# ActiveVisionLab/nope-nerf

Hardware: AMD Instinct MI355X
Metric: training rays/sec (higher is better)
Workload: dtype f32; 1 GPU; BASELINE configs[1]: 1024 rays/GPU x 192 samples, D=256, fp32 via three fp16 MFMA terms per product (fwd, dgrad, wgrad 4x4 + encoding tiles); fp32_products=split2, adam_arithmetic=single, rays_per_gpu=1024, total_rays=1024, n_samples=192, hidden=256, parallelism=dp1 (ray-sharded, one flat all-reduce)

## Files before the change

nope-nerf_amd/csrc/nnr_wgrad.hip:

```cpp
#include "nnr_device.h"
#include "nnr_kernels.h"
#include "nnr_split.h"
#include <cstdlib>

namespace nnr {

NNR_TL_DECL(tl_wgrad)
#ifdef NNR_TIMELINE
__device__ unsigned long long tl_wgrad_all[4096];
extern "C" int nnr_timeline_wgrad_all(unsigned long long* host4096) {
    return (int)hipMemcpyFromSymbol(host4096, HIP_SYMBOL(tl_wgrad_all), 4096 * sizeof(unsigned long long));
}
#endif

template <int W>
struct Vec { float v[W]; };

template <int W>
__device__ __forceinline__ Vec<W> load_vec(const float* p) {
    Vec<W> r;
    if constexpr (W == 4) {
        const f32x4 t = *reinterpret_cast<const f32x4*>(p);
        r.v[0] = t[0]; r.v[1] = t[1]; r.v[2] = t[2]; r.v[3] = t[3];
    } else if constexpr (W == 2) {
        const f32x2 t = *reinterpret_cast<const f32x2*>(p);
        r.v[0] = t[0]; r.v[1] = t[1];
    } else {
        r.v[0] = *p;
    }
    return r;
}

constexpr int kU = 4;
constexpr int32_t kPlanMagic = 0x4e4e5235;

template <int MI, int NI, int BIAS>
__device__ __forceinline__ void wgrad_job(const WgradJob& jb, const WgradArgs& a, int lane, int ji) {
    const int half = lane >> 5, m = lane & 31;
    const int dp = a.plane_pitch[jb.d_plane], xp = a.plane_pitch[jb.x_plane];
    const bool dok = MI * m < jb.d_valid, xok = NI * m < jb.x_valid;
    const bool dt = a.plane_tile[jb.d_plane] != 0, xt = a.plane_tile[jb.x_plane] != 0;
    const int dc = jb.d_col0 + (dok ? MI * m : 0), xc = jb.x_col0 + (xok ? NI * m : 0);
    const int d_row = dt ? 4 : dp, x_row = xt ? 4 : xp;
    const int64_t d_chunk = 32 * (int64_t)dp, x_chunk = 32 * (int64_t)xp;
    const float* dptr = a.ws + a.plane_off[jb.d_plane] + (dt ? (dc >> 3) * 256 + ((dc >> 2) & 1) * 128 + (dc & 3) : dc) + half * d_row;
    const float* xptr = a.ws + a.plane_off[jb.x_plane] + (xt ? (xc >> 3) * 256 + ((xc >> 2) & 1) * 128 + (xc & 3) : xc) + half * x_row;

    f32x16 acc[MI][NI];
#pragma unroll
    for (int i = 0; i < MI; ++i)
#pragma unroll
        for (int j = 0; j < NI; ++j)
#pragma unroll
            for (int r = 0; r < 16; ++r) acc[i][j][r] = 0.f;
    float bsum[MI];
#pragma unroll
    for (int i = 0; i < MI; ++i) bsum[i] = 0.f;

    Vec<MI> dA[kU], dB[kU];
    Vec<NI> xA[kU], xB[kU];
    auto load_stage = [&](Vec<MI>(&d)[kU], Vec<NI>(&x)[kU], int64_t kk) {
        const float* const dk = dptr + (kk >> 5) * d_chunk + (kk & 31) * d_row;
        const float* const xk = xptr + (kk >> 5) * x_chunk + (kk & 31) * x_row;
#pragma unroll
        for (int u = 0; u < kU; ++u) {
            d[u] = load_vec<MI>(dk + 2 * u * d_row);
            x[u] = load_vec<NI>(xk + 2 * u * x_row);
        }
    };
    auto compute = [&](const Vec<MI>(&d)[kU], const Vec<NI>(&x)[kU]) {
#pragma unroll
        for (int u = 0; u < kU; ++u) {
#pragma unroll
            for (int i = 0; i < MI; ++i) {
#pragma unroll
                for (int j = 0; j < NI; ++j) acc[i][j] = mfma32(d[u].v[i], x[u].v[j], acc[i][j]);
                if (BIAS == 1 || (BIAS == 2 && u % 2 == 0) || (BIAS == 3 && u % 2 == 1)) bsum[i] += d[u].v[i];
            }
        }
    };
    NNR_STAMP(tl_wgrad, 0);
    load_stage(dA, xA, jb.k0);
    for (int64_t k = jb.k0; k < jb.k1; k += 4 * kU) {
        load_stage(dB, xB, k + 2 * kU);
        __builtin_amdgcn_sched_barrier(0);
        compute(dA, xA);
        __builtin_amdgcn_sched_barrier(0);
        load_stage(dA, xA, (k + 4 * kU < jb.k1) ? k + 4 * kU : k);
        __builtin_amdgcn_sched_barrier(0);
        compute(dB, xB);
        __builtin_amdgcn_sched_barrier(0);
    }

    NNR_STAMP(tl_wgrad, 1);
#ifdef NNR_TIMELINE
    if (blockIdx.x == 700 / 8 && threadIdx.x == 0) { tl_wgrad[4] = (unsigned long long)(jb.k1 - jb.k0); tl_wgrad[5] = MI * 8 + NI; }
#endif
    float* slot = a.slots + (int64_t)ji * kSlotFloats;
#pragma unroll
    for (int i = 0; i < MI; ++i)
#pragma unroll
        for (int r = 0; r < 16; ++r) {
            const int mr = (r & 3) + 8 * (r >> 2) + 4 * half;
            float* dst = slot + (MI * mr + i) * (32 * NI) + NI * m;
            if constexpr (NI == 4) *reinterpret_cast<f32x4*>(dst) = f32x4{acc[i][0][r], acc[i][1][r], acc[i][2][r], acc[i][3][r]};
            else if constexpr (NI == 2) *reinterpret_cast<f32x2*>(dst) = f32x2{acc[i][0][r], acc[i][1][r]};
            else *dst = acc[i][0][r];
        }
    if constexpr (BIAS != 0) {
        float* dst = slot + kSlotTile + half * (32 * MI) + MI * m;
#pragma unroll
        for (int i = 0; i < MI; ++i) dst[i] = bsum[i];
    }
    NNR_STAMP(tl_wgrad, 2);
}

constexpr int kStageF4 = 2 * 16 * 64;

template <int BIAS, int NI, bool DTILE, bool XTILE>
__device__ __forceinline__ void wgrad_job_split(const WgradJob& jb, const WgradArgs& a, int lane, int ji, f32x4* stage) {
    constexpr int MI = 4;
    static_assert(NI == 4 || NI == 2, "activation sub-tiles per job");
    static_assert(!XTILE || NI == 4, "the tile-major activation image is laid out for whole 128-column tiles");
    constexpr int G = 6 * NI;
    static_assert(G >= 16, "block 3 issues the 16 DMA rows of the step after next, one per gap");
    const int half = lane >> 5, m = lane & 31;
    const int dp = a.plane_pitch[jb.d_plane], xp = a.plane_pitch[jb.x_plane];
    const bool dok = MI * m < jb.d_valid, xok = NI * m < jb.x_valid;
    const char* const dg = reinterpret_cast<const char*>(a.ws + a.plane_off[jb.d_plane] + (DTILE ? (jb.d_col0 >> 3) * 256 : jb.d_col0));
    const char* const xg = reinterpret_cast<const char*>(a.ws + a.plane_off[jb.x_plane] + (XTILE ? (jb.x_col0 >> 3) * 256 : jb.x_col0));
    const int tlane = ((lane & 15) >> 1) * 1024 + (lane & 1) * 512 + (lane >> 4) * 16;
    const int dlane = DTILE ? tlane : 4 * ((dok ? MI * m : 0) + 8 * half * dp);
    const int64_t d_chunk_bytes = 128 * (int64_t)dp, x_chunk_bytes = 128 * (int64_t)xp;
    const int xlane = XTILE ? tlane : NI == 4 ? 4 * ((xok ? NI * m : 0) + 8 * half * xp) : 4 * (4 * (m & 15) + 8 * half * xp);

    f32x16 acc[MI][NI];
#pragma unroll
    for (int i = 0; i < MI; ++i)
#pragma unroll
        for (int j = 0; j < NI; ++j)
#pragma unroll
            for (int r = 0; r < 16; ++r) acc[i][j][r] = 0.f;
    float bsum[MI] = {0.f, 0.f, 0.f, 0.f};
    uint32_t Xc[NI][3][4], Xn[NI][3][4], Dq[2][3][4];
    f32x2 fp[2][4];
    const float* const lrow = reinterpret_cast<const float*>(stage) + 4 * lane;
    const float* const lrowd = DTILE ? reinterpret_cast<const float*>(stage) + 4 * (256 * half + 64 * (m >> 4) + (m & 15)) : lrow;
    const float* const lrowx = XTILE ? reinterpret_cast<const float*>(stage) + 4 * (256 * half + 64 * (m >> 4) + (m & 15)) + 2048
                             : NI == 4 ? lrow : reinterpret_cast<const float*>(stage) + 4 * (32 * half + (m >> 1)) + 2 * (m & 1);

#define NNR_WDMA(G, LANE, P, KK, S, DST, ROW) \
    __builtin_amdgcn_global_load_lds((glb_ptr_t)((G) + ((KK) + (S)) * (int64_t)(P) * 4 + (LANE)), (lds_ptr_t)((DST) + (ROW) * 64), 16, 0, 0)
#define NNR_WPACK(V) __builtin_bit_cast(uint32_t, __builtin_convertvector(V, bf16x2))
#define NNR_WOFF(ROW0, P, C, SECOND) (((ROW0) == 0 ? DTILE : XTILE) ? 512 * ((P) >> 1) + 128 * ((P) & 1) + (C) + 64 * (SECOND) : 256 * ((ROW0) + 2 * (P) + (SECOND)) + (C))
#define NNR_WFETCH(W, P, LR, ROW0, C) (fp[W][P] = f32x2{(LR)[NNR_WOFF(ROW0, P, C, 0)], (LR)[NNR_WOFF(ROW0, P, C, 1)]})
#define NNR_WDMA_D(KK, S, DST, ROW)                                                                                                      \
    do {                                                                                                                                 \
        if constexpr (DTILE)                                                                                                             \
            __builtin_amdgcn_global_load_lds((glb_ptr_t)(dg + ((KK) >> 5) * d_chunk_bytes + ((KK) & 31) * 16 + ((S) & 1) * 8192 + ((S) >> 1) * 64 + dlane), \
                                             (lds_ptr_t)((DST) + (ROW) * 64), 16, 0, 0);                                                 \
        else NNR_WDMA(dg, dlane, dp, KK, S, DST, ROW);                                                                                    \
    } while (0)
#define NNR_WDMA_X(KK, S, DST, ROW)                                                                                                      \
    do {                                                                                                                                 \
        if constexpr (XTILE)                                                                                                             \
            __builtin_amdgcn_global_load_lds((glb_ptr_t)(xg + ((KK) >> 5) * x_chunk_bytes + ((KK) & 31) * 16 + ((S) & 1) * 8192 + ((S) >> 1) * 64 + xlane), \
                                             (lds_ptr_t)((DST) + (ROW) * 64), 16, 0, 0);                                                 \
        else NNR_WDMA(xg, xlane, xp, KK, S, DST, ROW);                                                                                    \
    } while (0)
#define NNR_WSPLIT(LR, ROW0, C, P, ST, Q, W, BI, BWT)                                        \
    do {                                                                                     \
        if ((ST) == 0) {                                                                     \
            NNR_WFETCH(W, P, LR, ROW0, C);                                                   \
        } else if ((ST) == 1) {                                                              \
            if ((BI) >= 0 && BIAS != 0)                                                      \
                bsum[(BI) >= 0 ? (BI) : 0] += (BWT) * (BIAS == 1 ? fp[W][P][0] + fp[W][P][1] : (BIAS == 2 ? fp[W][P][0] : fp[W][P][1])); \
            Q[2][P] = NNR_WPACK(fp[W][P]);                                   \
            fp[W][P] = pair_residual(fp[W][P], Q[2][P]);                                      \
        } else if ((ST) == 2) {                                                              \
            Q[1][P] = NNR_WPACK(fp[W][P]);                                   \
            fp[W][P] = pair_residual(fp[W][P], Q[1][P]);                                      \
        } else {                                                                             \
            Q[0][P] = NNR_WPACK(fp[W][P]);                                   \
        }                                                                                    \
    } while (0)
#define NNR_WSPLIT_ALL(LR, ROW0, C, Q, W, BI)                                                \
    _Pragma("unroll") for (int st_ = 0; st_ < 4; ++st_)                                      \
        _Pragma("unroll") for (int p_ = 0; p_ < 4; ++p_) NNR_WSPLIT(LR, ROW0, C, p_, st_, Q, W, BI, 1.f)

#pragma unroll
    for (int s = 0; s < 8; ++s) {
        NNR_WDMA_D((int64_t)jb.k0, s, stage, s);
        NNR_WDMA_X((int64_t)jb.k0, s, stage, 8 + s);
    }
    asm volatile("s_waitcnt vmcnt(0)" ::: "memory");
    {
        const int64_t k1st = jb.k0 + 16 < jb.k1 ? jb.k0 + 16 : jb.k0;
#pragma unroll
        for (int s = 0; s < 8; ++s) {
            NNR_WDMA_D(k1st, s, stage + 1024, s);
            NNR_WDMA_X(k1st, s, stage + 1024, 8 + s);
        }
    }
#pragma unroll
    for (int j = 0; j < NI; ++j) NNR_WSPLIT_ALL(lrowx, 8, j, Xc[j], 1, -1);
    NNR_WSPLIT_ALL(lrowd, 0, 0, Dq[0], 0, 0);

    for (int64_t k = jb.k0; k < jb.k1; k += 16) {
        const int par = (int)(((k - jb.k0) >> 4) & 1);
        const bool more = k + 16 < jb.k1;
        const int64_t kn = k + 32 < jb.k1 ? k + 32 : k;
        const float nf = more ? 1.f : 0.f;
        const float* const lc = lrowd + 4096 * par;
        const float* const ln = lrowd + 4096 * (1 - par);
        const float* const lnx = lrowx + 4096 * (1 - par);
        f32x4* const dst = stage + 1024 * par;
#pragma unroll
        for (int i = 0; i < MI; ++i) {
            if (i == 2) asm volatile("s_waitcnt vmcnt(0)" ::: "memory");
            constexpr int kXOps = 16 * (NI / 2);
            const int n_ops = 16 + (i >= 2 ? kXOps : 0);
            const int stride = n_ops / 16;
#pragma unroll
            for (int g = 0; g < G; ++g) {
                const int j = g / 6, t = g % 6;
                const int wc = t == 0 ? 0 : (t < 3 ? 1 : 2), xc = t == 0 ? 2 : (t == 1 ? 1 : (t == 2 ? 2 : t - 3));
                __builtin_amdgcn_sched_barrier(0);
                acc[i][j] = __builtin_amdgcn_mfma_f32_32x32x16_bf16(
                    __builtin_bit_cast(bf16x8, u32x4{Dq[i & 1][wc][0], Dq[i & 1][wc][1], Dq[i & 1][wc][2], Dq[i & 1][wc][3]}),
                    __builtin_bit_cast(bf16x8, u32x4{Xc[j][xc][0], Xc[j][xc][1], Xc[j][xc][2], Xc[j][xc][3]}),
                    acc[i][j], 0, 0, 0);
                __builtin_amdgcn_sched_barrier(0);
                {
                    const int q = i == 3 ? g : 16;
                    if (q < 8) NNR_WDMA_D(kn, q, dst, q);
                    else if (q < 16) NNR_WDMA_X(kn, q - 8, dst, q);
                }
#pragma unroll
                for (int o = 0; o < 48; ++o) {
                    if (o >= n_ops || (o * G) / n_ops != g) continue;
                    const bool is_d = stride == 1 || o % stride == 0;
                    const int od = stride == 1 ? o : o / stride, ox = o - o / stride - 1;
                    if (is_d) {
                        const int st = od / 4, p = od % 4;
                        if (i == 0) NNR_WSPLIT(lc, 0, 1, p, st, Dq[1], 0, 1, 1.f);
                        else if (i == 1) NNR_WSPLIT(lc, 0, 2, p, st, Dq[0], 0, 2, 1.f);
                        else if (i == 2) NNR_WSPLIT(lc, 0, 3, p, st, Dq[1], 0, 3, 1.f);
                        else NNR_WSPLIT(ln, 0, 0, p, st, Dq[0], 0, 0, nf);
                    } else {
                        const int cc = (NI / 2) * (i - 2) + ox / 16, r = ox % 16, st = r / 4, p = r % 4;
                        NNR_WSPLIT(lnx, 8, cc, p, st, Xn[cc], 1, -1, 0.f);
                    }
                }
            }
            if constexpr (NI == 4) asm volatile("" : "+a"(acc[i][0]), "+a"(acc[i][1]), "+a"(acc[i][2]), "+a"(acc[i][3]));
            else asm volatile("" : "+a"(acc[i][0]), "+a"(acc[i][1]));
        }
#pragma unroll
        for (int j = 0; j < NI; ++j)
#pragma unroll
            for (int t = 0; t < 3; ++t)
#pragma unroll
                for (int q = 0; q < 4; ++q) Xc[j][t][q] = Xn[j][t][q];
    }
    asm volatile("s_waitcnt vmcnt(0)" ::: "memory");
#undef NNR_WDMA
#undef NNR_WDMA_D
#undef NNR_WDMA_X
#undef NNR_WOFF
#undef NNR_WSPLIT
#undef NNR_WFETCH
#undef NNR_WPACK
#undef NNR_WSPLIT_ALL

    float* slot = a.slots + (int64_t)ji * kSlotFloats;
#pragma unroll
    for (int i = 0; i < MI; ++i)
#pragma unroll
        for (int r = 0; r < 16; ++r) {
            const int mr = (r & 3) + 8 * (r >> 2) + 4 * half;
            float* dst = slot + (MI * mr + i) * (32 * NI) + NI * m;
            if constexpr (NI == 4) *reinterpret_cast<f32x4*>(dst) = f32x4{acc[i][0][r], acc[i][1][r], acc[i][2][r], acc[i][3][r]};
            else *reinterpret_cast<f32x2*>(dst) = f32x2{acc[i][0][r], acc[i][1][r]};
        }
    if (jb.bias != 0) {
        float* dst = slot + kSlotTile + half * (32 * MI) + MI * m;
#pragma unroll
        for (int i = 0; i < MI; ++i) dst[i] = bsum[i];
    }
}

constexpr int kCoopStageF4 = 2 * 8 * 64;
constexpr int kCoopRegionF4 = 4 * 3 * 64;
constexpr int kCoopXchF4 = kWavesPerBlock * kCoopStageF4;
constexpr int kCoopF4 = kCoopXchF4 + 2 * 4 * kCoopRegionF4;

template <bool DTILE, bool XTILE>
__device__ __forceinline__ void wgrad_group_split(const WgradJob& jb, const WgradArgs& a, int lane, int ji, f32x4* lds_all, int wave) {
    constexpr int MI = 4, NI = 4;
    typedef uint32_t u32x2 __attribute__((ext_vector_type(2)));
    const int half = lane >> 5, m = lane & 31;
    const int ta = __builtin_amdgcn_readfirstlane(jb.d_col0 >> 7), tb = __builtin_amdgcn_readfirstlane(jb.x_col0 >> 7);
    const int dp = a.plane_pitch[jb.d_plane], xp = a.plane_pitch[jb.x_plane];
    f32x4* const stage = lds_all + wave * kCoopStageF4;
    const char* const dg = reinterpret_cast<const char*>(a.ws + a.plane_off[jb.d_plane] + (DTILE ? (jb.d_col0 >> 3) * 256 : jb.d_col0));
    const char* const xg = reinterpret_cast<const char*>(a.ws + a.plane_off[jb.x_plane] + (XTILE ? (jb.x_col0 >> 3) * 256 : jb.x_col0));
    const int tlane = ((lane & 15) >> 1) * 1024 + (lane & 1) * 512 + (lane >> 4) * 16;
    const int dlane = DTILE ? tlane : 4 * (MI * m + 8 * half * dp);
    const int xlane = XTILE ? tlane : 4 * (NI * m + 8 * half * xp);
    const int64_t d_chunk_bytes = 128 * (int64_t)dp, x_chunk_bytes = 128 * (int64_t)xp;
    auto dma_d = [&](int64_t KK, int r, f32x4* dst) __attribute__((always_inline)) {
        if constexpr (DTILE)
            __builtin_amdgcn_global_load_lds((glb_ptr_t)(dg + (KK >> 5) * d_chunk_bytes + (KK & 31) * 16 + (r & 1) * 8192 + (tb + 2 * (r >> 1)) * 64 + dlane),
                                             (lds_ptr_t)(dst + r * 64), 16, 0, 0);
        else
            __builtin_amdgcn_global_load_lds((glb_ptr_t)(dg + (KK + 4 * tb + r) * (int64_t)dp * 4 + dlane), (lds_ptr_t)(dst + r * 64), 16, 0, 0);
    };
    auto dma_x = [&](int64_t KK, int r, f32x4* dst) __attribute__((always_inline)) {
        if constexpr (XTILE)
            __builtin_amdgcn_global_load_lds((glb_ptr_t)(xg + (KK >> 5) * x_chunk_bytes + (KK & 31) * 16 + (r & 1) * 8192 + (ta + 2 * (r >> 1)) * 64 + xlane),
                                             (lds_ptr_t)(dst + (4 + r) * 64), 16, 0, 0);
        else
            __builtin_amdgcn_global_load_lds((glb_ptr_t)(xg + (KK + 4 * ta + r) * (int64_t)xp * 4 + xlane), (lds_ptr_t)(dst + (4 + r) * 64), 16, 0, 0);
    };
    const float* const sf = reinterpret_cast<const float*>(stage);
    const float* const lrd = DTILE ? sf + 4 * (128 * half + 64 * (m >> 4) + (m & 15)) : sf + 4 * lane;
    const float* const lrx = XTILE ? sf + 4 * (128 * half + 64 * (m >> 4) + (m & 15)) + 1024 : sf + 4 * lane;
    auto off_d = [](int pl, int C, int second) { return DTILE ? 128 * pl + C + 64 * second : 256 * (2 * pl + second) + C; };
    auto off_x = [](int pl, int C, int second) { return XTILE ? 128 * pl + C + 64 * second : 256 * (4 + 2 * pl + second) + C; };
    char* const xch = reinterpret_cast<char*>(lds_all + kCoopXchF4);
    constexpr int kBufBytes = 4 * kCoopRegionF4 * 16, kRegBytes = kCoopRegionF4 * 16;
    char* const rd_d = xch + ta * kRegBytes + lane * 16;
    char* const rd_x = xch + (2 + tb) * kRegBytes + lane * 16;
    char* const wr_d = rd_d + 8 * tb;
    char* const wr_x = rd_x + 8 * ta;

    f32x16 acc[MI][NI];
#pragma unroll
    for (int i = 0; i < MI; ++i)
#pragma unroll
        for (int j = 0; j < NI; ++j)
#pragma unroll
            for (int r = 0; r < 16; ++r) acc[i][j][r] = 0.f;
    float bsum[MI] = {0.f, 0.f, 0.f, 0.f};
    uint32_t Xc[NI][3][4], Dq[2][3][4];
    uint32_t T[4][3];
    f32x2 rr[4];

    auto pack = [](f32x2 v) { return __builtin_bit_cast(uint32_t, __builtin_convertvector(v, bf16x2)); };
    auto split_op = [&](int q, int st, const float* bd, const float* bx, float nf) __attribute__((always_inline)) {
        const int op = q >> 3, C = (q >> 1) & 3, pl = q & 1, s = q & 3;
        if (st == 0) {
            rr[s] = op == 0 ? f32x2{bd[off_d(pl, C, 0)], bd[off_d(pl, C, 1)]} : f32x2{bx[off_x(pl, C, 0)], bx[off_x(pl, C, 1)]};
        } else if (st == 1) {
            if (op == 0) bsum[C] += nf * (rr[s][0] + rr[s][1]);
            T[s][2] = pack(rr[s]);
            rr[s] = pair_residual(rr[s], T[s][2]);
        } else if (st == 2) {
            T[s][1] = pack(rr[s]);
            rr[s] = pair_residual(rr[s], T[s][1]);
        } else {
            T[s][0] = pack(rr[s]);
        }
    };
    auto write_op = [&](int op, int C, int t, int eb) __attribute__((always_inline)) {
        char* const p = (op == 0 ? wr_d : wr_x) + eb * kBufBytes + ((C * 3 + t) * 64) * 16;
        *reinterpret_cast<u32x2*>(p) = u32x2{T[2 * (C & 1)][t], T[2 * (C & 1) + 1][t]};
    };
    auto read_terms = [&](uint32_t (&dst)[3][4], const char* base, int sub, int eb) __attribute__((always_inline)) {
#pragma unroll
        for (int t = 0; t < 3; ++t) {
            const u32x4 v = *reinterpret_cast<const u32x4*>(base + eb * kBufBytes + ((sub * 3 + t) * 64) * 16);
            dst[t][0] = v[0]; dst[t][1] = v[1]; dst[t][2] = v[2]; dst[t][3] = v[3];
        }
    };
    auto coop_op = [&](int n, const float* bd, const float* bx, float nf, int eb) __attribute__((always_inline)) {
        const int B = n / 22, o = n % 22;
        if (o < 16) split_op(4 * B + (o & 3), o >> 2, bd, bx, nf);
        else write_op(B >> 1, 2 * (B & 1) + (o - 16) / 3, (o - 16) % 3, eb);
    };

    asm volatile("s_waitcnt vmcnt(0) lgkmcnt(0)" ::: "memory");
    __builtin_amdgcn_s_barrier();
#pragma unroll
    for (int r = 0; r < 4; ++r) {
        dma_d(jb.k0, r, stage);
        dma_x(jb.k0, r, stage);
    }
    asm volatile("s_waitcnt vmcnt(0)" ::: "memory");
    {
        const int64_t k1st = jb.k0 + 16 < jb.k1 ? jb.k0 + 16 : jb.k0;
#pragma unroll
        for (int r = 0; r < 4; ++r) {
            dma_d(k1st, r, stage + 512);
            dma_x(k1st, r, stage + 512);
        }
    }
#pragma unroll
    for (int n = 0; n < 88; ++n) coop_op(n, lrd, lrx, 1.f, 0);
    asm volatile("s_waitcnt lgkmcnt(0)" ::: "memory");
    __builtin_amdgcn_s_barrier();
#pragma unroll
    for (int j = 0; j < NI; ++j) read_terms(Xc[j], rd_x, j, 0);
    read_terms(Dq[0], rd_d, 0, 0);

    for (int64_t k = jb.k0; k < jb.k1; k += 16) {
        const int e = (int)(((k - jb.k0) >> 4) & 1);
        const bool more = k + 16 < jb.k1;
        const int64_t kn = k + 32 < jb.k1 ? k + 32 : k;
        const float nf = more ? 1.f : 0.f;
        const float* const bd = lrd + 2048 * (1 - e);
        const float* const bx = lrx + 2048 * (1 - e);
        f32x4* const dst = stage + 512 * e;
        asm volatile("s_waitcnt vmcnt(0)" ::: "memory");
#pragma unroll
        for (int i = 0; i < MI; ++i) {
            if (i == 3) {
                asm volatile("s_waitcnt lgkmcnt(0)" ::: "memory");
                __builtin_amdgcn_s_barrier();
            }
#pragma unroll
            for (int g = 0; g < 24; ++g) {
                const int j = g / 6, t = g % 6;
                const int wc = t == 0 ? 0 : (t < 3 ? 1 : 2), xc = t == 0 ? 2 : (t == 1 ? 1 : (t == 2 ? 2 : t - 3));
                __builtin_amdgcn_sched_barrier(0);
                acc[i][j] = __builtin_amdgcn_mfma_f32_32x32x16_bf16(
                    __builtin_bit_cast(bf16x8, u32x4{Dq[i & 1][wc][0], Dq[i & 1][wc][1], Dq[i & 1][wc][2], Dq[i & 1][wc][3]}),
                    __builtin_bit_cast(bf16x8, u32x4{Xc[j][xc][0], Xc[j][xc][1], Xc[j][xc][2], Xc[j][xc][3]}),
                    acc[i][j], 0, 0, 0);
                __builtin_amdgcn_sched_barrier(0);
                if (i < 3) {
                    const int gg = 24 * i + g;
                    if (g == 1) read_terms(Dq[(i + 1) & 1], rd_d, i + 1, e);
                    if (i == 0 && g >= 4 && g < 12) {
                        if (g < 8) dma_d(kn, g - 4, dst);
                        else dma_x(kn, g - 8, dst);
                    }
#pragma unroll
                    for (int n = 0; n < 88; ++n)
                        if ((n * 72) / 88 == gg) coop_op(n, bd, bx, nf, 1 - e);
                } else {
                    if (t == 5) read_terms(Xc[j], rd_x, j, 1 - e);
                    if (g == 20) read_terms(Dq[0], rd_d, 0, 1 - e);
                }
            }
            asm volatile("" : "+a"(acc[i][0]), "+a"(acc[i][1]), "+a"(acc[i][2]), "+a"(acc[i][3]));
        }
    }
    asm volatile("s_waitcnt vmcnt(0) lgkmcnt(0)" ::: "memory");

    float* slot = a.slots + (int64_t)ji * kSlotFloats;
#pragma unroll
    for (int i = 0; i < MI; ++i)
#pragma unroll
        for (int r = 0; r < 16; ++r) {
            const int mr = (r & 3) + 8 * (r >> 2) + 4 * half;
            float* dst = slot + (MI * mr + i) * (32 * NI) + NI * m;
            *reinterpret_cast<f32x4*>(dst) = f32x4{acc[i][0][r], acc[i][1][r], acc[i][2][r], acc[i][3][r]};
        }
    if (jb.bias != 0) {
        float* dst = slot + kSlotTile + half * (32 * MI) + MI * m;
#pragma unroll
        for (int i = 0; i < MI; ++i) dst[i] = bsum[i];
    }
}

constexpr int kCoop2RegionF4 = 4 * 2 * 64;
constexpr int kCoop2F4 = kCoopXchF4 + 2 * 4 * kCoop2RegionF4;

__device__ __forceinline__ float plane_scale(float mx) {
    const int eb = (int)((__float_as_uint(mx) >> 23) & 255u);
    int es = 267 - eb;
    es = es > 227 ? 227 : (es < 27 ? 27 : es);
    return mx > 0.f ? __uint_as_float((uint32_t)es << 23) : 1.f;
}

template <bool DTILE, bool XTILE>
__device__ __forceinline__ void wgrad_group_split2(const WgradJob& jb, const WgradArgs& a, int lane, int ji, f32x4* lds_all, int wave) {
    constexpr int MI = 4, NI = 4;
    typedef uint32_t u32x2 __attribute__((ext_vector_type(2)));
    typedef _Float16 f16x2 __attribute__((ext_vector_type(2)));
    typedef _Float16 f16x8 __attribute__((ext_vector_type(8)));
    const int half = lane >> 5, m = lane & 31;
    const int ta = __builtin_amdgcn_readfirstlane(jb.d_col0 >> 7), tb = __builtin_amdgcn_readfirstlane(jb.x_col0 >> 7);
    const int dp = a.plane_pitch[jb.d_plane], xp = a.plane_pitch[jb.x_plane];
    f32x4* const stage = lds_all + wave * kCoopStageF4;
    const float sd = plane_scale(a.plane_max[jb.d_plane == P_DG ? 16 : 8 + (jb.d_plane - P_DH1)]);
    const float sx = plane_scale(a.plane_max[jb.x_plane - P_XH1]);
    const char* const dg = reinterpret_cast<const char*>(a.ws + a.plane_off[jb.d_plane] + (DTILE ? (jb.d_col0 >> 3) * 256 : jb.d_col0));
    const char* const xg = reinterpret_cast<const char*>(a.ws + a.plane_off[jb.x_plane] + (XTILE ? (jb.x_col0 >> 3) * 256 : jb.x_col0));
    const int tlane = ((lane & 15) >> 1) * 1024 + (lane & 1) * 512 + (lane >> 4) * 16;
    const int dlane = DTILE ? tlane : 4 * (MI * m + 8 * half * dp);
    const int xlane = XTILE ? tlane : 4 * (NI * m + 8 * half * xp);
    const int64_t d_chunk_bytes = 128 * (int64_t)dp, x_chunk_bytes = 128 * (int64_t)xp;
    auto dma_d = [&](int64_t KK, int r, f32x4* dst) __attribute__((always_inline)) {
        if constexpr (DTILE)
            __builtin_amdgcn_global_load_lds((glb_ptr_t)(dg + (KK >> 5) * d_chunk_bytes + (KK & 31) * 16 + (r & 1) * 8192 + (tb + 2 * (r >> 1)) * 64 + dlane),
                                             (lds_ptr_t)(dst + r * 64), 16, 0, 0);
        else
            __builtin_amdgcn_global_load_lds((glb_ptr_t)(dg + (KK + 4 * tb + r) * (int64_t)dp * 4 + dlane), (lds_ptr_t)(dst + r * 64), 16, 0, 0);
    };
    auto dma_x = [&](int64_t KK, int r, f32x4* dst) __attribute__((always_inline)) {
        if constexpr (XTILE)
            __builtin_amdgcn_global_load_lds((glb_ptr_t)(xg + (KK >> 5) * x_chunk_bytes + (KK & 31) * 16 + (r & 1) * 8192 + (ta + 2 * (r >> 1)) * 64 + xlane),
                                             (lds_ptr_t)(dst + (4 + r) * 64), 16, 0, 0);
        else
            __builtin_amdgcn_global_load_lds((glb_ptr_t)(xg + (KK + 4 * ta + r) * (int64_t)xp * 4 + xlane), (lds_ptr_t)(dst + (4 + r) * 64), 16, 0, 0);
    };
    const float* const sf = reinterpret_cast<const float*>(stage);
    const float* const lrd = DTILE ? sf + 4 * (128 * half + 64 * (m >> 4) + (m & 15)) : sf + 4 * lane;
    const float* const lrx = XTILE ? sf + 4 * (128 * half + 64 * (m >> 4) + (m & 15)) + 1024 : sf + 4 * lane;
    auto off_d = [](int pl, int C, int second) { return DTILE ? 128 * pl + C + 64 * second : 256 * (2 * pl + second) + C; };
    auto off_x = [](int pl, int C, int second) { return XTILE ? 128 * pl + C + 64 * second : 256 * (4 + 2 * pl + second) + C; };
    char* const xch = reinterpret_cast<char*>(lds_all + kCoopXchF4);
    constexpr int kBufBytes = 4 * kCoop2RegionF4 * 16, kRegBytes = kCoop2RegionF4 * 16;
    char* const rd_d = xch + ta * kRegBytes + lane * 16;
    char* const rd_x = xch + (2 + tb) * kRegBytes + lane * 16;
    char* const wr_d = rd_d + 8 * tb;
    char* const wr_x = rd_x + 8 * ta;

    f32x16 acc[MI][NI];
#pragma unroll
    for (int i = 0; i < MI; ++i)
#pragma unroll
        for (int j = 0; j < NI; ++j)
#pragma unroll
            for (int r = 0; r < 16; ++r) acc[i][j][r] = 0.f;
    float bsum[MI] = {0.f, 0.f, 0.f, 0.f};
    uint32_t Xc[NI][3][4], Dq[2][3][4];
    auto down11 = [](uint32_t (&t)[3][4]) __attribute__((always_inline)) {
        const f16x8 v = __builtin_bit_cast(f16x8, u32x4{t[1][0], t[1][1], t[1][2], t[1][3]}) * (_Float16)0.00048828125f;
        const u32x4 u = __builtin_bit_cast(u32x4, v);
        t[2][0] = u[0]; t[2][1] = u[1]; t[2][2] = u[2]; t[2][3] = u[3];
    };
    uint32_t T[4][2];
    f32x2 rr[4];

    auto split_op = [&](int q, int st, const float* bd, const float* bx, float nf) __attribute__((always_inline)) {
        const int op = q >> 3, C = (q >> 1) & 3, pl = q & 1, s = q & 3;
        if (st == 0) {
            rr[s] = op == 0 ? f32x2{bd[off_d(pl, C, 0)], bd[off_d(pl, C, 1)]} : f32x2{bx[off_x(pl, C, 0)], bx[off_x(pl, C, 1)]};
        } else if (st == 1) {
            if (op == 0) bsum[C] += nf * (rr[s][0] + rr[s][1]);
            rr[s] = rr[s] * (op == 0 ? sd : sx);
            const f16x2 hh = __builtin_convertvector(rr[s], f16x2);
            T[s][1] = __builtin_bit_cast(uint32_t, hh);
            rr[s] = (rr[s] - __builtin_convertvector(hh, f32x2)) * 2048.f;
        } else {
            T[s][0] = __builtin_bit_cast(uint32_t, __builtin_convertvector(rr[s], f16x2));
        }
    };
    auto write_op = [&](int op, int C, int t, int eb) __attribute__((always_inline)) {
        char* const p = (op == 0 ? wr_d : wr_x) + eb * kBufBytes + ((C * 2 + t) * 64) * 16;
        *reinterpret_cast<u32x2*>(p) = u32x2{T[2 * (C & 1)][t], T[2 * (C & 1) + 1][t]};
    };
    auto read_terms = [&](uint32_t (&dst)[3][4], const char* base, int sub, int eb) __attribute__((always_inline)) {
#pragma unroll
        for (int t = 0; t < 2; ++t) {
            const u32x4 v = *reinterpret_cast<const u32x4*>(base + eb * kBufBytes + ((sub * 2 + t) * 64) * 16);
            dst[t][0] = v[0]; dst[t][1] = v[1]; dst[t][2] = v[2]; dst[t][3] = v[3];
        }
    };
    auto coop_op = [&](int n, const float* bd, const float* bx, float nf, int eb) __attribute__((always_inline)) {
        const int B = n / 16, o = n % 16;
        if (o < 12) split_op(4 * B + (o & 3), o >> 2, bd, bx, nf);
        else write_op(B >> 1, 2 * (B & 1) + (o - 12) / 2, (o - 12) % 2, eb);
    };

    asm volatile("s_waitcnt vmcnt(0) lgkmcnt(0)" ::: "memory");
    __builtin_amdgcn_s_barrier();
#pragma unroll
    for (int r = 0; r < 4; ++r) {
        dma_d(jb.k0, r, stage);
        dma_x(jb.k0, r, stage);
    }
    asm volatile("s_waitcnt vmcnt(0)" ::: "memory");
    {
        const int64_t k1st = jb.k0 + 16 < jb.k1 ? jb.k0 + 16 : jb.k0;
#pragma unroll
        for (int r = 0; r < 4; ++r) {
            dma_d(k1st, r, stage + 512);
            dma_x(k1st, r, stage + 512);
        }
    }
#pragma unroll
    for (int n = 0; n < 64; ++n) coop_op(n, lrd, lrx, 1.f, 0);
    asm volatile("s_waitcnt lgkmcnt(0)" ::: "memory");
    __builtin_amdgcn_s_barrier();
#pragma unroll
    for (int j = 0; j < NI; ++j) { read_terms(Xc[j], rd_x, j, 0); down11(Xc[j]); }
    read_terms(Dq[0], rd_d, 0, 0);
    down11(Dq[0]);

    for (int64_t k = jb.k0; k < jb.k1; k += 16) {
        const int e = (int)(((k - jb.k0) >> 4) & 1);
        const bool more = k + 16 < jb.k1;
        const int64_t kn = k + 32 < jb.k1 ? k + 32 : k;
        const float nf = more ? 1.f : 0.f;
        const float* const bd = lrd + 2048 * (1 - e);
        const float* const bx = lrx + 2048 * (1 - e);
        f32x4* const dst = stage + 512 * e;
        asm volatile("s_waitcnt vmcnt(0)" ::: "memory");
#pragma unroll
        for (int i = 0; i < MI; ++i) {
            if (i == 3) {
                asm volatile("s_waitcnt lgkmcnt(0)" ::: "memory");
                __builtin_amdgcn_s_barrier();
            }
#pragma unroll
            for (int g = 0; g < 12; ++g) {
                if (i == 0 && g == 1 && k != jb.k0) down11(Xc[3]);
                const int j = g / 3, t = g % 3;
                const int wc = t == 0 ? 0 : (t == 1 ? 2 : 1), xc = t == 0 ? 2 : (t == 1 ? 0 : 1);
                __builtin_amdgcn_sched_barrier(0);
                acc[i][j] = __builtin_amdgcn_mfma_f32_32x32x16_f16(
                    __builtin_bit_cast(f16x8, u32x4{Dq[i & 1][wc][0], Dq[i & 1][wc][1], Dq[i & 1][wc][2], Dq[i & 1][wc][3]}),
                    __builtin_bit_cast(f16x8, u32x4{Xc[j][xc][0], Xc[j][xc][1], Xc[j][xc][2], Xc[j][xc][3]}),
                    acc[i][j], 0, 0, 0);
                __builtin_amdgcn_sched_barrier(0);
                if (i < 3) {
                    const int gg = 12 * i + g;
                    if (g == 1) read_terms(Dq[(i + 1) & 1], rd_d, i + 1, e);
                    if (g == 7) down11(Dq[(i + 1) & 1]);
                    if (i == 0 && g >= 4 && g < 12) {
                        if (g < 8) dma_d(kn, g - 4, dst);
                        else dma_x(kn, g - 8, dst);
                    }
#pragma unroll
                    for (int n = 0; n < 64; ++n)
                        if ((n * 36) / 64 == gg) coop_op(n, bd, bx, nf, 1 - e);
                } else {
                    if (t == 2) read_terms(Xc[j], rd_x, j, 1 - e);
                    if (t == 2 && j > 0) down11(Xc[j - 1]);
                    if (g == 3) read_terms(Dq[0], rd_d, 0, 1 - e);
                    if (g == 9) down11(Dq[0]);
                }
            }
            asm volatile("" : "+a"(acc[i][0]), "+a"(acc[i][1]), "+a"(acc[i][2]), "+a"(acc[i][3]));
        }
    }
    asm volatile("s_waitcnt vmcnt(0) lgkmcnt(0)" ::: "memory");

    float* slot = a.slots + (int64_t)ji * kSlotFloats;
#pragma unroll
    for (int i = 0; i < MI; ++i)
#pragma unroll
        for (int r = 0; r < 16; ++r) {
            const int mr = (r & 3) + 8 * (r >> 2) + 4 * half;
            float* dst = slot + (MI * mr + i) * (32 * NI) + NI * m;
            *reinterpret_cast<f32x4*>(dst) = f32x4{acc[i][0][r], acc[i][1][r], acc[i][2][r], acc[i][3][r]};
        }
    if (jb.bias != 0) {
        float* dst = slot + kSlotTile + half * (32 * MI) + MI * m;
#pragma unroll
        for (int i = 0; i < MI; ++i) dst[i] = bsum[i];
    }
}

#if defined(NNR_TIMELINE) && !defined(NNR_WGRAD_F16_TU)
extern "C" int nnr_timeline_wgrad(unsigned long long* host32) {
    return (int)hipMemcpyFromSymbol(host32, HIP_SYMBOL(tl_wgrad), 32 * sizeof(unsigned long long));
}
#endif

constexpr int kEncRows = 12;
constexpr int kEncStageF4 = 3 * kEncRows * 64;
constexpr int kPlaneMaxEnc = 17;

__device__ __forceinline__ void wgrad_job_enc2(const WgradJob& jb, const WgradArgs& a, int lane, int ji, f32x4* stage) {
    constexpr int MI = 4, NI = 2;
    typedef _Float16 f16x2 __attribute__((ext_vector_type(2)));
    typedef _Float16 f16x8 __attribute__((ext_vector_type(8)));
    const int half = lane >> 5, m = lane & 31;
    const int dp = a.plane_pitch[jb.d_plane], xp = a.plane_pitch[jb.x_plane];
    const float sd = plane_scale(a.plane_max[8 + (jb.d_plane - P_DH1)]);
    const float sx = plane_scale(a.plane_max[kPlaneMaxEnc]);
    const char* const dg = reinterpret_cast<const char*>(a.ws + a.plane_off[jb.d_plane] + (jb.d_col0 >> 3) * 256);
    const char* const xg = reinterpret_cast<const char*>(a.ws + a.plane_off[jb.x_plane] + (jb.x_col0 >> 3) * 256);
    const int tlane = ((lane & 15) >> 1) * 1024 + (lane & 1) * 512 + (lane >> 4) * 16;
    const int64_t d_chunk_bytes = 128 * (int64_t)dp, x_chunk_bytes = 128 * (int64_t)xp;
    auto dma_step = [&](int64_t KK, f32x4* dst) __attribute__((always_inline)) {
        const char* const dk = dg + (KK >> 5) * d_chunk_bytes + (KK & 31) * 16 + tlane;
        const char* const xk = xg + (KK >> 5) * x_chunk_bytes + (KK & 31) * 16 + tlane;
#pragma unroll
        for (int S = 0; S < 8; ++S)
            __builtin_amdgcn_global_load_lds((glb_ptr_t)(dk + (S & 1) * 8192 + (S >> 1) * 64), (lds_ptr_t)(dst + S * 64), 16, 0, 0);
#pragma unroll
        for (int S = 0; S < 4; ++S)
            __builtin_amdgcn_global_load_lds((glb_ptr_t)(xk + S * 64), (lds_ptr_t)(dst + (8 + S) * 64), 16, 0, 0);
    };
    const int base_d = 4 * (256 * half + 64 * (m >> 4) + (m & 15));
    const int base_x = 4 * (8 * 64) + 512 * half + 4 * (m >> 1) + 2 * (m & 1);
    auto off_d = [](int P, int C, int second) { return 512 * (P >> 1) + 128 * (P & 1) + 64 * second + C; };
    auto off_x = [](int P, int J, int second) { return 256 * (P >> 1) + 128 * (P & 1) + 64 * second + J; };

    f32x16 acc[MI][NI];
#pragma unroll
    for (int i = 0; i < MI; ++i)
#pragma unroll
        for (int j = 0; j < NI; ++j)
#pragma unroll
            for (int r = 0; r < 16; ++r) acc[i][j][r] = 0.f;
    float bsum[MI] = {0.f, 0.f, 0.f, 0.f};
    auto down11 = [](u32x4 h) __attribute__((always_inline)) {
        return __builtin_bit_cast(u32x4, __builtin_bit_cast(f16x8, h) * (_Float16)0.00048828125f);
    };
    auto split = [](f32x2 v, float sc, uint32_t& h, uint32_t& mm) __attribute__((always_inline)) {
        v = v * sc;
        const f16x2 hh = __builtin_convertvector(v, f16x2);
        h = __builtin_bit_cast(uint32_t, hh);
        mm = __builtin_bit_cast(uint32_t, __builtin_convertvector((v - __builtin_convertvector(hh, f32x2)) * 2048.f, f16x2));
    };

    const int64_t n_steps = (jb.k1 - jb.k0) >> 4;
    auto step_at = [&](int64_t t) { return jb.k0 + 16 * (t < n_steps ? t : n_steps - 1); };
    f32x4 dv[8];
    f32x2 ev[8];
    u32x4 Eh[NI], Em[NI], Es[NI];
    u32x4 Dh, Dm, Ds, Nh, Nm;
    auto load_rows = [&](int b) __attribute__((always_inline)) {
        const float* const sf = reinterpret_cast<const float*>(stage + b * (kEncRows * 64));
#pragma unroll
        for (int q = 0; q < 8; ++q) {
            dv[q] = *reinterpret_cast<const f32x4*>(sf + base_d + off_d(q >> 1, 0, q & 1));
            ev[q] = *reinterpret_cast<const f32x2*>(sf + base_x + off_x(q >> 1, 0, q & 1));
        }
    };
    auto split_e = [&](int j, int P) __attribute__((always_inline)) {
        uint32_t h, mm;
        split(f32x2{ev[2 * P][j], ev[2 * P + 1][j]}, sx, h, mm);
        Eh[j][P] = h; Em[j][P] = mm;
    };
    auto split_d = [&](int i, int P, u32x4& H, u32x4& M, float wb = 1.f) __attribute__((always_inline)) {
        const f32x2 v = {dv[2 * P][i], dv[2 * P + 1][i]};
        bsum[i] += wb * (v[0] + v[1]);
        uint32_t h, mm;
        split(v, sd, h, mm);
        H[P] = h; M[P] = mm;
    };
    asm volatile("s_waitcnt vmcnt(0) lgkmcnt(0)" ::: "memory");
    dma_step(step_at(0), stage);
    dma_step(step_at(1), stage + kEncRows * 64);
    asm volatile("s_waitcnt vmcnt(12)" ::: "memory");
    load_rows(0);
#pragma unroll
    for (int j = 0; j < NI; ++j) {
#pragma unroll
        for (int P = 0; P < 4; ++P) split_e(j, P);
        Es[j] = down11(Eh[j]);
    }
#pragma unroll
    for (int P = 0; P < 4; ++P) split_d(0, P, Dh, Dm);
    Ds = down11(Dh);
    for (int64_t t = 0; t < n_steps; ++t) {
        const int b = (int)(t % 3);
        dma_step(step_at(t + 2), stage + ((b + 2) % 3) * (kEncRows * 64));
        u32x4 Enh[NI], Enm[NI];
#pragma unroll
        for (int i = 0; i < MI; ++i) {
#pragma unroll
            for (int g = 0; g < 6; ++g) {
                const int j = g / 3, tt = g % 3;
                __builtin_amdgcn_sched_barrier(0);
                acc[i][j] = __builtin_amdgcn_mfma_f32_32x32x16_f16(__builtin_bit_cast(f16x8, tt == 0 ? Dm : (tt == 1 ? Ds : Dh)),
                                                                 __builtin_bit_cast(f16x8, tt == 0 ? Es[j] : (tt == 1 ? Em[j] : Eh[j])), acc[i][j], 0, 0, 0);
                __builtin_amdgcn_sched_barrier(0);
                if (i < 3) {
                    if (g < 4) split_d(i + 1, g, Nh, Nm);
                } else {
                    if (g == 0) {
                        asm volatile("s_waitcnt vmcnt(12)" ::: "memory");
                        load_rows((b + 1) % 3);
                    } else if (g < 5) {
                        const int q = 2 * (g - 1);
                        uint32_t h, mm;
                        split(f32x2{ev[2 * (q & 3)][q >> 2], ev[2 * (q & 3) + 1][q >> 2]}, sx, h, mm);
                        Enh[q >> 2][q & 3] = h; Enm[q >> 2][q & 3] = mm;
                        split(f32x2{ev[2 * ((q + 1) & 3)][(q + 1) >> 2], ev[2 * ((q + 1) & 3) + 1][(q + 1) >> 2]}, sx, h, mm);
                        Enh[(q + 1) >> 2][(q + 1) & 3] = h; Enm[(q + 1) >> 2][(q + 1) & 3] = mm;
                    }
                }
            }
            asm volatile("" : "+a"(acc[i][0]), "+a"(acc[i][1]));
            if (i < 3) {
                Dh = Nh; Dm = Nm;
                Ds = down11(Dh);
            }
        }
        const float keep = t + 1 < n_steps ? 1.f : 0.f;
#pragma unroll
        for (int P = 0; P < 4; ++P) split_d(0, P, Dh, Dm, keep);
        Ds = down11(Dh);
#pragma unroll
        for (int j = 0; j < NI; ++j) {
            Eh[j] = Enh[j]; Em[j] = Enm[j];
            Es[j] = down11(Eh[j]);
        }
    }
    asm volatile("s_waitcnt vmcnt(0)" ::: "memory");

    float* slot = a.slots + (int64_t)ji * kSlotFloats;
#pragma unroll
    for (int i = 0; i < MI; ++i)
#pragma unroll
        for (int r = 0; r < 16; ++r) {
            const int mr = (r & 3) + 8 * (r >> 2) + 4 * half;
            float* dst = slot + (MI * mr + i) * (32 * NI) + NI * m;
            *reinterpret_cast<f32x2*>(dst) = f32x2{acc[i][0][r], acc[i][1][r]};
        }
    if (jb.bias != 0) {
        float* dst = slot + kSlotTile + half * (32 * MI) + MI * m;
#pragma unroll
        for (int i = 0; i < MI; ++i) dst[i] = bsum[i];
    }
}

template <bool SPLIT, bool F16 = false>
__global__ __launch_bounds__(256, 1) void wgrad_kernel(WgradArgs a) {
    constexpr int kLdsBase = kCoopF4 > kWavesPerBlock * kStageF4 ? kCoopF4 : kWavesPerBlock * kStageF4;
    __shared__ __attribute__((aligned(16))) f32x4 stage_all[SPLIT ? (F16 && kWavesPerBlock * kEncStageF4 > kLdsBase ? kWavesPerBlock * kEncStageF4 : kLdsBase) : 1];
    const int lane = threadIdx.x & 63;
    const int wslot = __builtin_amdgcn_readfirstlane(blockIdx.x * 4 + (threadIdx.x >> 6));
    {
        const int32_t* const tr = a.heads + a.n_heads;
        if (tr[0] != kPlanMagic || tr[1] != a.n_jobs || tr[2] != a.n_waves || tr[3] != a.n_heads) __builtin_trap();
    }
    const int j0 = a.wave_first[wslot], j1 = a.wave_first[wslot + 1];
    if (blockIdx.x == 0) {
        for (int l = 0; l < 13; ++l)
            for (int r = threadIdx.x; r < a.bias_rows[l]; r += 256) a.gb[l][r] = 0.f;
    }
#ifdef NNR_TIMELINE
    if (lane == 0 && wslot < 2048) tl_wgrad_all[2 * wslot] = __builtin_amdgcn_s_memtime();
#endif
    for (int ji = j0; ji < j1; ++ji) {
        const WgradJob jb = a.jobs[ji];
        const int key = __builtin_amdgcn_readfirstlane(jb.MI * 8 + jb.NI + 64 * jb.bias);
#define NNR_WGRAD_RUN(MI_, NI_, B_) wgrad_job<MI_, NI_, B_>(jb, a, lane, ji)
#define NNR_WGRAD_CASE(MI_, NI_)                                 \
    case MI_ * 8 + NI_: NNR_WGRAD_RUN(MI_, NI_, 0); break;        \
    case MI_ * 8 + NI_ + 64: NNR_WGRAD_RUN(MI_, NI_, 1); break;
        if constexpr (SPLIT) {
            if (__builtin_amdgcn_readfirstlane(jb.reserved) == 1) {
                if constexpr (F16)
                    wgrad_group_split2<kTileGradPlanes, kTileActPlanes>(jb, a, lane, ji, stage_all, __builtin_amdgcn_readfirstlane((int)(threadIdx.x >> 6)));
                else
                    wgrad_group_split<kTileGradPlanes, kTileActPlanes>(jb, a, lane, ji, stage_all, __builtin_amdgcn_readfirstlane((int)(threadIdx.x >> 6)));
                continue;
            }
            if constexpr (F16) {
                if (__builtin_amdgcn_readfirstlane(jb.reserved) == 2) {
                    wgrad_job_enc2(jb, a, lane, ji, stage_all + __builtin_amdgcn_readfirstlane((int)(threadIdx.x >> 6)) * kEncStageF4);
                    continue;
                }
            }
            if (__builtin_amdgcn_readfirstlane(jb.MI * 8 + jb.NI) == 4 * 8 + 4) {
                constexpr int kPrivateF4 = F16 && kEncStageF4 > kStageF4 ? kEncStageF4 : kStageF4;
                static_assert(kWavesPerBlock * kPrivateF4 <= (int)(sizeof(stage_all) / sizeof(f32x4)), "the four private staging areas fit in stage_all");
                f32x4* const stage = stage_all + __builtin_amdgcn_readfirstlane((int)(threadIdx.x >> 6)) * kPrivateF4;
                switch (__builtin_amdgcn_readfirstlane(jb.bias)) {
                    case 2: wgrad_job_split<2, 4, kTileGradPlanes, kTileActPlanes>(jb, a, lane, ji, stage); break;
                    case 3: wgrad_job_split<3, 4, kTileGradPlanes, kTileActPlanes>(jb, a, lane, ji, stage); break;
                    default: wgrad_job_split<1, 4, kTileGradPlanes, kTileActPlanes>(jb, a, lane, ji, stage); break;
                }
                continue;
            }
        }
        switch (key) {
            case 4 * 8 + 4 + 128: NNR_WGRAD_RUN(4, 4, 2); break;
            case 4 * 8 + 4 + 192: NNR_WGRAD_RUN(4, 4, 3); break;
            NNR_WGRAD_CASE(4, 4)
            NNR_WGRAD_CASE(4, 2)
            NNR_WGRAD_CASE(4, 1)
            NNR_WGRAD_CASE(2, 4)
            NNR_WGRAD_CASE(2, 1)
            NNR_WGRAD_CASE(1, 4)
            NNR_WGRAD_CASE(1, 2)
            default: break;
        }
#undef NNR_WGRAD_CASE
#undef NNR_WGRAD_RUN
    }
#ifdef NNR_TIMELINE
    if (lane == 0 && wslot < 2048) tl_wgrad_all[2 * wslot + 1] = __builtin_amdgcn_s_memtime();
#endif
}

hipError_t launch_wgrad_f16_main(const WgradArgs& a, hipStream_t st);
#ifdef NNR_WGRAD_F16_TU
hipError_t launch_wgrad_f16_main(const WgradArgs& a, hipStream_t st) {
    hipLaunchKernelGGL((wgrad_kernel<true, true>), dim3(a.n_waves / 4), dim3(256), 0, st, a);
    return hipGetLastError();
}
#else
constexpr int kMaxChain = 256;
__global__ __launch_bounds__(256) void wgrad_reduce_kernel(WgradArgs a) {
    const int ji = a.heads[blockIdx.x >> 4];
    const WgradJob jb = a.jobs[ji];
    __shared__ int chain[kMaxChain];
    __shared__ int n_chain;
    if (threadIdx.x == 0) {
        int n = 0, j = ji;
        for (; j >= 0 && n < kMaxChain; j = a.jobs[j].next_split) chain[n++] = j - ji;
        if (j >= 0) __builtin_trap();
        n_chain = n;
    }
    __syncthreads();
    const int n = n_chain;
    const int t = (blockIdx.x & 15) * 256 + threadIdx.x;
    const int pitch = 32 * jb.NI, f4_per_row = 8 * jb.NI;
    const int row = t / f4_per_row, c0 = 4 * (t - row * f4_per_row);
    if (row < 32 * jb.MI && row < jb.d_valid && jb.row0 + row < jb.rows_real) {
        f32x4 sum = {0.f, 0.f, 0.f, 0.f};
        const float* src = a.slots + (int64_t)ji * kSlotFloats + row * pitch + c0;
        int s = 0;
        for (; s + 8 <= n; s += 8) {
            f32x4 v[8];
#pragma unroll
            for (int u = 0; u < 8; ++u) v[u] = *reinterpret_cast<const f32x4*>(src + (int64_t)chain[s + u] * kSlotFloats);
#pragma unroll
            for (int u = 0; u < 8; ++u) sum += v[u];
        }
        for (; s < n; ++s) sum += *reinterpret_cast<const f32x4*>(src + (int64_t)chain[s] * kSlotFloats);
        if (a.plane_max != nullptr && jb.reserved == 2) {
            const float sd = plane_scale(a.plane_max[8 + (jb.d_plane - P_DH1)]), sx = plane_scale(a.plane_max[kPlaneMaxEnc]);
            sum = (sum * (1.f / sd)) * (1.f / sx);
        }
        if (a.plane_max != nullptr && jb.reserved == 1) {
            const float sd = plane_scale(a.plane_max[jb.d_plane == P_DG ? 16 : 8 + (jb.d_plane - P_DH1)]), sx = plane_scale(a.plane_max[jb.x_plane - P_XH1]);
            sum = (sum * (1.f / sd)) * (1.f / sx);
        }
        float* dst = a.gw[jb.layer] + (int64_t)(jb.row0 + row) * jb.ldw + jb.wcol0 + c0;
#pragma unroll
        for (int e = 0; e < 4; ++e)
            if (c0 + e < jb.x_valid && jb.wcol0 + c0 + e < jb.cols_real) dst[e] = sum[e];
    }
    if (jb.bias && (blockIdx.x & 15) == 0 && (int)threadIdx.x < 32 * jb.MI) {
        const int r = threadIdx.x;
        if (r < jb.d_valid && jb.row0 + r < jb.rows_real) {
            float sum = 0.f;
            const float* src = a.slots + (int64_t)ji * kSlotFloats + kSlotTile + r;
            for (int s = 0; s < n; ++s) {
                const float* p = src + (int64_t)chain[s] * kSlotFloats;
                sum += p[0] + p[32 * jb.MI];
            }
            atomicAdd(a.gb[jb.layer] + jb.row0 + r, sum);
        }
    }
}

template <int D, int BF16>
__global__ __launch_bounds__(256) void wgrad_unmerge_kernel(WgradArgs a) {
    using L = Layout<D, BF16>;
    constexpr int Dh = L::Dh, ldg = D + kDirReal;
    const float* Wf = a.packed + L::copy_wf_off;
    const float* Wg1 = a.packed + L::copy_wg_off;
    const float* bf = a.packed + L::copy_bf_off;
    const float* dWm = a.gw[kMergedLayer];
    const float* dbm = a.gb[kMergedLayer];
    const int gid = blockIdx.x * 256 + threadIdx.x;
    if (gid < D * D) {
        const int j = gid / D, k = gid - j * D;
        float acc = 0.f;
#pragma unroll 16
        for (int m = 0; m < Dh; ++m) acc = fmaf(Wg1[m * D + j], dWm[m * D + k], acc);
        a.gw[9][gid] = acc;
    } else if (gid < D * D + Dh * D) {
        const int t = gid - D * D, m = t / D, j = t - m * D;
        float acc = dbm[m] * bf[j];
#pragma unroll 16
        for (int k = 0; k < D; ++k) acc = fmaf(dWm[m * D + k], Wf[j * D + k], acc);
        a.gw[10][m * ldg + j] = acc;
    } else if (gid < D * D + Dh * D + D) {
        const int j = gid - D * D - Dh * D;
        float acc = 0.f;
        for (int m = 0; m < Dh; ++m) acc = fmaf(Wg1[m * D + j], dbm[m], acc);
        a.gb[9][j] = acc;
    } else if (gid < D * D + Dh * D + D + Dh) {
        const int m = gid - D * D - Dh * D - D;
        a.gb[10][m] = dbm[m];
    }
}

hipError_t launch_wgrad(const WgradArgs& a, hipStream_t st) {
    hipError_t e;
    prof_before(PROF_WGRAD, st);
    static const bool split_off = std::getenv("NNR_WGRAD_FP32") != nullptr;
    static const bool f16_off = std::getenv("NNR_WGRAD_BF16_TERMS") != nullptr;
    WgradArgs b = a;
    if (!(a.bf16 == 3 && a.plane_max != nullptr && !split_off && !f16_off)) b.plane_max = nullptr;
    if (b.plane_max != nullptr) (void)launch_wgrad_f16_main(b, st);
    else if (a.bf16 >= 2 && !split_off) hipLaunchKernelGGL(wgrad_kernel<true>, dim3(a.n_waves / 4), dim3(256), 0, st, b);
    else hipLaunchKernelGGL(wgrad_kernel<false>, dim3(a.n_waves / 4), dim3(256), 0, st, b);
    hipLaunchKernelGGL(wgrad_reduce_kernel, dim3(a.n_heads * 16), dim3(256), 0, st, b);
    e = hipGetLastError();
    if (e == hipSuccess) e = launch_wgrad_unmerge(a, st);
    prof_after(PROF_WGRAD, st);
    return e;
}

hipError_t launch_wgrad_unmerge(const WgradArgs& a, hipStream_t st) {
    const int threads = a.D * a.D + (a.D / 2) * a.D + a.D + a.D / 2;
    const dim3 grid((threads + 255) / 256), block(256);
    if (a.D == 256) {
        if (a.bf16 == 3) hipLaunchKernelGGL((wgrad_unmerge_kernel<256, 3>), grid, block, 0, st, a);
        else if (a.bf16 == 2) hipLaunchKernelGGL((wgrad_unmerge_kernel<256, 2>), grid, block, 0, st, a);
        else if (a.bf16 == 1) hipLaunchKernelGGL((wgrad_unmerge_kernel<256, 1>), grid, block, 0, st, a);
        else hipLaunchKernelGGL((wgrad_unmerge_kernel<256, 0>), grid, block, 0, st, a);
    } else {
        if (a.bf16 == 3) hipLaunchKernelGGL((wgrad_unmerge_kernel<128, 3>), grid, block, 0, st, a);
        else if (a.bf16 == 2) hipLaunchKernelGGL((wgrad_unmerge_kernel<128, 2>), grid, block, 0, st, a);
        else if (a.bf16 == 1) hipLaunchKernelGGL((wgrad_unmerge_kernel<128, 1>), grid, block, 0, st, a);
        else hipLaunchKernelGGL((wgrad_unmerge_kernel<128, 0>), grid, block, 0, st, a);
    }
    return hipGetLastError();
}

#endif

}
```

Baseline: 448,200 rays/s.

## Triple-buffer global-to-LDS staging in split2 wgrad group job

Deepens the per-wave global_load_lds staging ring in the two-term wgrad workgroup job from two buffers to three. DMA for tile k+48 is issued while tile k is consumed, and the per-iteration wait becomes a partial vmcnt instead of a full drain, to hide global memory latency. The LDS exchange region is moved to fit inside the existing stage allocation, checked by a static_assert. Optional timeline instrumentation macros are also added, compiled out by default.

After: 438,600 rays/s. 0.979x the previous value.

```diff
diff --git a/nope-nerf_amd/csrc/nnr_wgrad.hip b/nope-nerf_amd/csrc/nnr_wgrad.hip
--- a/nope-nerf_amd/csrc/nnr_wgrad.hip
+++ b/nope-nerf_amd/csrc/nnr_wgrad.hip
@@ -465,8 +465,12 @@
     }
 }
 
+constexpr int kCoop2Bufs = 3;
+constexpr int kCoop2StageF4 = kCoop2Bufs * 8 * 64;
+constexpr int kCoop2XchF4 = kWavesPerBlock * kCoop2StageF4;
 constexpr int kCoop2RegionF4 = 4 * 2 * 64;
-constexpr int kCoop2F4 = kCoopXchF4 + 2 * 4 * kCoop2RegionF4;
+constexpr int kCoop2F4 = kCoop2XchF4 + 2 * 4 * kCoop2RegionF4;
+static_assert(kCoop2F4 == kCoopF4, "the two-term workgroup job takes exactly the 160 KiB stage_all is sized for (the six-term job's footprint)");
 
 __device__ __forceinline__ float plane_scale(float mx) {
     const int eb = (int)((__float_as_uint(mx) >> 23) & 255u);
@@ -474,6 +478,41 @@
     es = es > 227 ? 227 : (es < 27 ? 27 : es);
     return mx > 0.f ? __uint_as_float((uint32_t)es << 23) : 1.f;
 }
+
+#if defined(NNR_TIMELINE) && defined(NNR_WGRAD_F16_TU)
+constexpr int kTlGroupJobs = 4096;
+__device__ unsigned long long tl_wgrad_group[kTlGroupJobs * 6];
+extern "C" int nnr_timeline_wgrad_group(unsigned long long* host) {
+    return (int)hipMemcpyFromSymbol(host, HIP_SYMBOL(tl_wgrad_group), sizeof(tl_wgrad_group));
+}
+#define NNR_COOP2_TL_BEGIN                                                                                            \
+    unsigned long long tl_wait = 0, tl_req = 0, tl_a = 0, tl_b = 0, tl_c = 0, tl_d = 0;                               \
+    const unsigned long long tl_t0 = __builtin_amdgcn_s_memtime(), tl_r0 = __builtin_amdgcn_s_memrealtime();
+#define NNR_COOP2_TL_WAIT0 tl_a = __builtin_amdgcn_s_memtime();
+#define NNR_COOP2_TL_WAIT1                     \
+    tl_b = __builtin_amdgcn_s_memtime();       \
+    tl_req += tl_d - tl_c;                     \
+    tl_wait += tl_b - tl_a;
+#define NNR_COOP2_TL_REQ0 tl_c = __builtin_amdgcn_s_memtime();
+#define NNR_COOP2_TL_REQ1 tl_d = __builtin_amdgcn_s_memtime();
+#define NNR_COOP2_TL_END                                                                                  \
+    if (lane == 0 && wave == 0 && ji < kTlGroupJobs) {                                                    \
+        unsigned long long* const o = tl_wgrad_group + 6 * ji;                                            \
+        o[0] = (unsigned long long)((jb.k1 - jb.k0) >> 4);                                                \
+        o[1] = __builtin_amdgcn_s_memtime() - tl_t0;                                                      \
+        o[2] = tl_wait;                                                                                   \
+        o[3] = tl_req + (tl_d - tl_c);                                                                    \
+        o[4] = __builtin_amdgcn_s_memrealtime() - tl_r0;                                                  \
+        o[5] = (unsigned long long)blockIdx.x;                                                            \
+    }
+#else
+#define NNR_COOP2_TL_BEGIN
+#define NNR_COOP2_TL_WAIT0
+#define NNR_COOP2_TL_WAIT1
+#define NNR_COOP2_TL_REQ0
+#define NNR_COOP2_TL_REQ1
+#define NNR_COOP2_TL_END
+#endif
 
 template <bool DTILE, bool XTILE>
 __device__ __forceinline__ void wgrad_group_split2(const WgradJob& jb, const WgradArgs& a, int lane, int ji, f32x4* lds_all, int wave) {
@@ -484,7 +523,7 @@
     const int half = lane >> 5, m = lane & 31;
     const int ta = __builtin_amdgcn_readfirstlane(jb.d_col0 >> 7), tb = __builtin_amdgcn_readfirstlane(jb.x_col0 >> 7);
     const int dp = a.plane_pitch[jb.d_plane], xp = a.plane_pitch[jb.x_plane];
-    f32x4* const stage = lds_all + wave * kCoopStageF4;
+    f32x4* const stage = lds_all + wave * kCoop2StageF4;
     const float sd = plane_scale(a.plane_max[jb.d_plane == P_DG ? 16 : 8 + (jb.d_plane - P_DH1)]);
     const float sx = plane_scale(a.plane_max[jb.x_plane - P_XH1]);
     const char* const dg = reinterpret_cast<const char*>(a.ws + a.plane_off[jb.d_plane] + (DTILE ? (jb.d_col0 >> 3) * 256 : jb.d_col0));
@@ -512,7 +551,7 @@
     const float* const lrx = XTILE ? sf + 4 * (128 * half + 64 * (m >> 4) + (m & 15)) + 1024 : sf + 4 * lane;
     auto off_d = [](int pl, int C, int second) { return DTILE ? 128 * pl + C + 64 * second : 256 * (2 * pl + second) + C; };
     auto off_x = [](int pl, int C, int second) { return XTILE ? 128 * pl + C + 64 * second : 256 * (4 + 2 * pl + second) + C; };
-    char* const xch = reinterpret_cast<char*>(lds_all + kCoopXchF4);
+    char* const xch = reinterpret_cast<char*>(lds_all + kCoop2XchF4);
     constexpr int kBufBytes = 4 * kCoop2RegionF4 * 16, kRegBytes = kCoop2RegionF4 * 16;
     char* const rd_d = xch + ta * kRegBytes + lane * 16;
     char* const rd_x = xch + (2 + tb) * kRegBytes + lane * 16;
@@ -570,19 +609,15 @@
     asm volatile("s_waitcnt vmcnt(0) lgkmcnt(0)" ::: "memory");
     __builtin_amdgcn_s_barrier();
 #pragma unroll
-    for (int r = 0; r < 4; ++r) {
-        dma_d(jb.k0, r, stage);
-        dma_x(jb.k0, r, stage);
-    }
-    asm volatile("s_waitcnt vmcnt(0)" ::: "memory");
-    {
-        const int64_t k1st = jb.k0 + 16 < jb.k1 ? jb.k0 + 16 : jb.k0;
+    for (int b = 0; b < kCoop2Bufs; ++b) {
+        const int64_t kb = jb.k0 + 16 * b < jb.k1 ? jb.k0 + 16 * b : jb.k0;
 #pragma unroll
         for (int r = 0; r < 4; ++r) {
-            dma_d(k1st, r, stage + 512);
-            dma_x(k1st, r, stage + 512);
-        }
-    }
+            dma_d(kb, r, stage + 512 * b);
+            dma_x(kb, r, stage + 512 * b);
+        }
+    }
+    asm volatile("s_waitcnt vmcnt(%0)" ::"n"(8 * (kCoop2Bufs - 1)) : "memory");
 #pragma unroll
     for (int n = 0; n < 64; ++n) coop_op(n, lrd, lrx, 1.f, 0);
     asm volatile("s_waitcnt lgkmcnt(0)" ::: "memory");
@@ -592,15 +627,20 @@
     read_terms(Dq[0], rd_d, 0, 0);
     down11(Dq[0]);
 
+    NNR_COOP2_TL_BEGIN
+    int sb = 0;
     for (int64_t k = jb.k0; k < jb.k1; k += 16) {
         const int e = (int)(((k - jb.k0) >> 4) & 1);
+        const int sn = sb + 1 == kCoop2Bufs ? 0 : sb + 1;
         const bool more = k + 16 < jb.k1;
-        const int64_t kn = k + 32 < jb.k1 ? k + 32 : k;
+        const int64_t kn = k + 16 * kCoop2Bufs < jb.k1 ? k + 16 * kCoop2Bufs : k;
         const float nf = more ? 1.f : 0.f;
-        const float* const bd = lrd + 2048 * (1 - e);
-        const float* const bx = lrx + 2048 * (1 - e);
-        f32x4* const dst = stage + 512 * e;
-        asm volatile("s_waitcnt vmcnt(0)" ::: "memory");
+        const float* const bd = lrd + 2048 * sn;
+        const float* const bx = lrx + 2048 * sn;
+        f32x4* const dst = stage + 512 * sb;
+        NNR_COOP2_TL_WAIT0
+        asm volatile("s_waitcnt vmcnt(%0)" ::"n"(8 * (kCoop2Bufs - 2)) : "memory");
+        NNR_COOP2_TL_WAIT1
 #pragma unroll
         for (int i = 0; i < MI; ++i) {
             if (i == 3) {
@@ -618,14 +658,16 @@
                     __builtin_bit_cast(f16x8, u32x4{Xc[j][xc][0], Xc[j][xc][1], Xc[j][xc][2], Xc[j][xc][3]}),
                     acc[i][j], 0, 0, 0);
                 __builtin_amdgcn_sched_barrier(0);
+                if (i == 0 && g >= 4 && g < 12) {
+                    if (g == 4) { NNR_COOP2_TL_REQ0 }
+                    if (g < 8) dma_d(kn, g - 4, dst);
+                    else dma_x(kn, g - 8, dst);
+                    if (g == 11) { NNR_COOP2_TL_REQ1 }
+                }
                 if (i < 3) {
                     const int gg = 12 * i + g;
                     if (g == 1) read_terms(Dq[(i + 1) & 1], rd_d, i + 1, e);
                     if (g == 7) down11(Dq[(i + 1) & 1]);
-                    if (i == 0 && g >= 4 && g < 12) {
-                        if (g < 8) dma_d(kn, g - 4, dst);
-                        else dma_x(kn, g - 8, dst);
-                    }
 #pragma unroll
                     for (int n = 0; n < 64; ++n)
                         if ((n * 36) / 64 == gg) coop_op(n, bd, bx, nf, 1 - e);
@@ -638,7 +680,9 @@
             }
             asm volatile("" : "+a"(acc[i][0]), "+a"(acc[i][1]), "+a"(acc[i][2]), "+a"(acc[i][3]));
         }
-    }
+        sb = sn;
+    }
+    NNR_COOP2_TL_END
     asm volatile("s_waitcnt vmcnt(0) lgkmcnt(0)" ::: "memory");
 
     float* slot = a.slots + (int64_t)ji * kSlotFloats;
```
